# cropinghigh/sdrpp-dvbs-demodulator

Measured on NVIDIA B200. Metric: decoded_info_gbit_s, higher is better.
Workload: dtype int8

## Files before the change

sdrpp-dvbs-demodulator_b200/csrc/ldpc_v2.cuh:

```cuda
#pragma once
#include "ldpc_decoder.cuh"
#include "ldpc_variants.h"

#include <type_traits>

namespace s2 {
namespace v2 {

constexpr int kThreads = 360;

__device__ __forceinline__ uint32_t prmt(uint32_t a, uint32_t b, uint32_t sel) {
    uint32_t d;
    asm("prmt.b32 %0, %1, %2, %3;" : "=r"(d) : "r"(a), "r"(b), "r"(sel));
    return d;
}
__device__ __forceinline__ uint32_t minu2(uint32_t a, uint32_t b) {
    uint32_t d;
    asm("min.u16x2 %0, %1, %2;" : "=r"(d) : "r"(a), "r"(b));
    return d;
}
__device__ __forceinline__ uint32_t min3u2(uint32_t a, uint32_t b, uint32_t c) {
    uint32_t d;
    asm("{.reg .b32 t; min.u16x2 t, %1, %2; min.u16x2 %0, t, %3;}" : "=r"(d) : "r"(a), "r"(b), "r"(c));
    return d;
// ... 242 lines not shown
    const int8_t* ptB = inB + K;
    const int cols = min(360, (K / q) & ~7);
    const int jj = tid % 360, i0 = tid / 360;
    for (int j0 = 0; j0 < 360; j0 += cols) {
        const int nc = min(cols, 360 - j0);
        const int b8 = q * j0 / 8;
        for (int x = tid; x < q * nc / 8; x += THREADS) v4[x] = interleave8(ld_in8<STREAMED>(ptA, b8 + x), ld_in8<STREAMED>(ptB, b8 + x));
        __syncthreads();
        if (jj < nc)
            for (int i = i0; i < q; i += THREADS / 360) __stcg(&wpty[i * 360 + j0 + jj], vdata[jj * q + i]);
        __syncthreads();
    }
    for (int x = tid; x < K / 8; x += THREADS) v4[x] = interleave8(ld_in8<STREAMED>(inA, x), ld_in8<STREAMED>(inB, x));
}

constexpr unsigned kNoPair = 0xFFFFFFFFu;
template <bool STREAMED>
__device__ __noinline__ unsigned claim_next_pair(const LdpcParams2& p, unsigned npairs) {
    if (*reinterpret_cast<const volatile unsigned*>(p.work_counter) + gridDim.x >= npairs) return kNoPair;
    const unsigned np = atomicAdd(p.work_counter, 1u);
    if (np < npairs) {
        const unsigned f0 = 2u * np, nf = min(2u, (unsigned)p.nframes - f0);
        if (!STREAMED || *reinterpret_cast<const volatile unsigned*>(p.arrived) >= f0 + nf) {
            const size_t b = reinterpret_cast<size_t>(p.llr_in + (size_t)f0 * p.N);
            const size_t lo = b & ~(size_t)15, hi = (b + (size_t)nf * p.N + 15) & ~(size_t)15;
            asm volatile("cp.async.bulk.prefetch.L2.global [%0], %1;" ::"l"(lo), "r"((unsigned)(hi - lo)) : "memory");
        }
    }
    return np;
}

static __device__ __noinline__ bool wait_arrived(const unsigned int* arrived_ptr, unsigned need, long long budget) {
    const volatile unsigned* arrived = arrived_ptr;
    const long long t0 = clock64();
    while (*arrived < need) {
        __nanosleep(500);
        if (clock64() - t0 > budget) return false;
    }
    return true;
}

template <int CNT, bool RAGGED, bool STREAMED, int OCC>
__global__ void __launch_bounds__(kThreads, OCC) ldpc_v2_kernel(const __grid_constant__ LdpcParams2 p) {
    constexpr int SLOTS = CNT + 2;
    constexpr int MW = (SLOTS + 1) / 2;
    constexpr int SG = (SLOTS + 7) / 8;
    static_assert(16 * SG >= 2 * SLOTS + 2, "the message record needs two spare bytes (row level)");
    constexpr int DW = (1 + 2 * CNT + 3) & ~3;
    extern __shared__ __align__(16) uint8_t smem_raw[];
    const int q = p.q, K = p.K, N = p.N, R = p.R;
    uint16_t* vdata = reinterpret_cast<uint16_t*>(smem_raw);
    uint16_t* X = reinterpret_cast<uint16_t*>(smem_raw + (size_t)K * 2);
    uint32_t* desc = reinterpret_cast<uint32_t*>(smem_raw + (size_t)K * 2 + 768);
    __shared__ unsigned int s_pair;
    __shared__ int s_bad[2];

    const int tid = threadIdx.x;
    const int j = tid;
    const uint32_t vbase = (uint32_t)__cvta_generic_to_shared(vdata);
    uint32_t dbase = (uint32_t)__cvta_generic_to_shared(desc);
    uint32_t j2 = 2u * (uint32_t)j;
    uint32_t xaddr = (uint32_t)__cvta_generic_to_shared(X) + j2;
    uint32_t m1 = 0xFFFFFFFFu;
    uint4* wmsg = reinterpret_cast<uint4*>(p.workspace + (size_t)blockIdx.x * p.ws_stride);
    uint16_t* wpty = reinterpret_cast<uint16_t*>(p.workspace + (size_t)blockIdx.x * p.ws_stride + (size_t)q * SG * 360 * 16);
    uint32_t* HD = reinterpret_cast<uint32_t*>(reinterpret_cast<uint8_t*>(wpty) + (((size_t)R * 2 + 15) & ~(size_t)15));
    uint32_t* HP = HD + 2 * p.ngroups * kBitWords;
    {
        volatile uint4* opq = reinterpret_cast<volatile uint4*>(HP + 2 * q * kBitWords + 4) + tid;
// ... 1 lines not shown
        j2 = opq->x; xaddr = opq->y; dbase = opq->z; m1 = opq->w;
    }
    for (int x = tid; x < q * DW; x += kThreads) {
        const int i = x / DW, w = x - i * DW;
        const int loff = p.layer_off[i], cnt = (int)p.layer_off[i + 1] - loff;
        uint32_t v = 0;
        if (w == 0) {
            v = (uint32_t)p.layer_nlev[i] | (uint32_t)p.layer_sync[i] << 8 | (uint32_t)cnt << 16;
        } else if (w <= 2 * CNT) {
            const int c = (w - 1) >> 1;
            const int k = loff + (c < cnt ? c : 0);
            v = ((w - 1) & 1) ? (uint32_t)p.link_add[k] : vbase + 720u * p.link_group[k];
        }
        desc[x] = v;
    }
    const int npairs = (p.nframes + 1) >> 1;

    for (int x = tid; x < 2 * (p.ngroups + q) * kBitWords; x += kThreads) __stcg(&HD[x], 0u);
    __shared__ unsigned int s_next;
    if (tid == 0) s_next = kNoPair;

    for (;;) {
        __syncthreads();
        if (tid == 0) {
            unsigned np = s_next;
            if (np == kNoPair) np = atomicAdd(p.work_counter, 1u);
            s_next = kNoPair;
            if (STREAMED && np < (unsigned)npairs) {
                if (!wait_arrived(p.arrived, min(2u * np + 2u, (unsigned)p.nframes), p.wait_budget)) np |= 0x80000000u;
                __threadfence();
            }
            s_pair = np;
        }
        __syncthreads();
        const unsigned pair_word = s_pair;
        const unsigned pair = pair_word & 0x7FFFFFFFu;
        if (pair >= (unsigned)npairs) break;
        const int fa = 2 * pair, fb = 2 * pair + 1;
        const bool hasB = fb < p.nframes;
        if (STREAMED && (pair_word & 0x80000000u)) {
            if (tid == 0) {
                p.iters_out[fa] = kLdpcItersNoInput;
                if (hasB) p.iters_out[fb] = kLdpcItersNoInput;
            }
            continue;
        }
        const int8_t* inA = p.llr_in + (size_t)fa * N;
        const int8_t* inB = p.llr_in + (size_t)(hasB ? fb : fa) * N;

        load_pair<STREAMED, kThreads>(p, inA, inB, vdata, wpty);
        uint32_t pown = 0, psec = 0;
        {
            const uint32_t last = __ldcg(wpty + (q - 1) * 360 + j);
            X[j + 1] = (uint16_t)last;
            pown = unpack_lo(last);
            psec = unpack_lo(__ldcg(wpty + (q - 2) * 360 + j));
        }
        if (tid == 0) X[0] = 0xFFFFu;

        int live = hasB ? 3 : 1;
        uint32_t off[CNT];
        uint32_t lw0 = 0;
        auto link_addresses = [&](int i) {
            uint32_t dw[DW];
#pragma unroll
            for (int x = 0; x < DW; x += 4)
                asm volatile("ld.shared.v4.u32 {%0, %1, %2, %3}, [%4];" : "=r"(dw[x]), "=r"(dw[x + 1]), "=r"(dw[x + 2]), "=r"(dw[x + 3])
                             : "r"(dbase + (uint32_t)(i * DW + x) * 4u));
            lw0 = dw[0];
#pragma unroll
            for (int c = 0; c < CNT; ++c)
                off[c] = dw[1 + 2 * c] + addmin_u32(j2 + dw[2 + 2 * c], (uint32_t)-720);
        };
        auto screen = [&]() -> int {
            link_addresses(q - 1);
            const int cnt = (int)(lw0 >> 16);
            uint32_t sx = pown ^ psec, mn = minu2(__vabsdiffu4(pown, kC128), __vabsdiffu4(psec, kC128));
            int nl = 2;
#pragma unroll
            for (int c = 0; c < CNT; ++c) {
                if (!RAGGED || c < cnt) {
                    const uint32_t u = unpack_lo(lds_u16(off[c]));
                    sx ^= u;
                    mn = minu2(mn, __vabsdiffu4(u, kC128));
                    ++nl;
                }
            }
            if (nl & 1) sx ^= kC128;
            int bad = 0;
            if ((sx & 0x80u) || (mn & 0xFFFFu) == 0) bad |= 1;
            if ((sx & 0x800000u) || (mn >> 16) == 0) bad |= 2;
            return bad;
        };

        __syncthreads();
        int scr = screen();
        int res[2] = {-1, -1};
        for (int n = 0;; ++n) {
            int bad = (__syncthreads_or(scr & 1) ? 1 : 0) | (__syncthreads_or(scr & 2) ? 2 : 0);
            if (live & ~bad)
                bad = full_test<kThreads>(p, wpty, HP, HD, reinterpret_cast<const uint4*>(vdata), s_bad);
            int fin = 0;
            for (int f = 0; f < 2; ++f) {
                if (!(live >> f & 1)) continue;
                if (!(bad >> f & 1)) {
                    res[f] = n;
                    fin |= 1 << f;
                } else if (n == p.max_trials) {
                    fin |= 1 << f;
                }
            }
            if (fin) {
                emit_results<kThreads>(p, fin, res, fa, fb, wpty, reinterpret_cast<const uint4*>(vdata));
                if (tid == 0 && s_next == kNoPair) s_next = claim_next_pair<STREAMED>(p, (unsigned)npairs);
                live &= ~fin;
                if (live) __syncthreads();
            }
            if (!live) break;

            auto pass = [&](auto first_tag) {
                constexpr bool FIRST = decltype(first_tag)::value;
                uint32_t mw[MW];
                uint4 nxt[SG];
                uint32_t pnext = 0;
                uint32_t pprev = 0;
#pragma unroll
                for (int x = 0; x < MW; ++x) mw[x] = 0;
                uint4* rp = wmsg + j;
                uint16_t* pp = wpty + j;
                psec = unpack_lo(lds_u16(xaddr));
                pnext = __ldcg(pp);
                if (!FIRST) {
#pragma unroll
                    for (int s = 0; s < SG; ++s) nxt[s] = __ldcg(rp + s * 360);
                }
                uint32_t lev_next = (FIRST && p.layer_nlev[0] > 1) ? (uint32_t)p.row_level[j] << 24 : 0u;
                for (int i = 0; i < q; ++i) {
                    uint32_t keep = lev_next;
                    if (!FIRST) {
#pragma unroll
                        for (int s = 0; s < SG; ++s) {
                            if (4 * s + 0 < MW) mw[4 * s + 0] = nxt[s].x;
                            if (4 * s + 1 < MW) mw[4 * s + 1] = nxt[s].y;
                            if (4 * s + 2 < MW) mw[4 * s + 2] = nxt[s].z;
                            if (4 * s + 3 < MW) mw[4 * s + 3] = nxt[s].w;
                        }
                        keep = nxt[SG - 1].w;
                    }
                    pown = unpack_lo(i == q - 1 ? lds_u16(xaddr + 2) : pnext);
                    if (i + 1 < q) {
                        pnext = __ldcg(pp + 360);
                        if (!FIRST) {
#pragma unroll
                            for (int s = 0; s < SG; ++s) nxt[s] = __ldcg(rp + (SG + s) * 360);
                        }
                    }
                    link_addresses(i);
                    const int cnt = RAGGED ? (int)(lw0 >> 16) : CNT;
                    const int nlev = (int)(lw0 & 0xFFu);
                    if (FIRST) lev_next = (i + 1 < q && p.layer_nlev[i + 1] > 1) ? (uint32_t)p.row_level[(i + 1) * 360 + j] << 24 : 0u;
                    if (nlev == 1) {
                        row_update<CNT, FIRST, RAGGED>(off, cnt, mw, pown, psec, keep, m1);
                        if (lw0 & 0x100u) __syncthreads();
                    } else {
                        const int mylev = (int)(keep >> 24);
                        for (int lvl = 0; lvl < nlev; ++lvl) {
                            if (mylev == lvl) row_update<CNT, FIRST, RAGGED>(off, cnt, mw, pown, psec, keep, m1);
                            __syncthreads();
                        }
                    }
#pragma unroll
                    for (int s = 0; s < SG; ++s) {
                        uint4 o;
                        o.x = (4 * s + 0 < MW) ? mw[4 * s + 0] : 0u;
                        o.y = (4 * s + 1 < MW) ? mw[4 * s + 1] : 0u;
                        o.z = (4 * s + 2 < MW) ? mw[4 * s + 2] : 0u;
                        o.w = (4 * s + 3 < MW) ? mw[4 * s + 3] : 0u;
                        if (s == SG - 1 && 4 * s + 3 >= MW) o.w = keep & 0xFF000000u;
                        __stcg(rp + s * 360, o);
                    }
                    if (i == 0)
                        sts_u16(xaddr, pack_pair(psec));
                    else
                        __stcg(pp - 360, (uint16_t)pack_pair(psec));
                    pprev = psec;
                    psec = pown;
                    rp += SG * 360;
                    pp += 360;
                }
                psec = pprev;
                {
                    const uint16_t pk = (uint16_t)pack_pair(pown);
                    sts_u16(xaddr + 2, pk);
                    __stcg(pp - 360, pk);
                }
            };
            if (n == 0) pass(std::true_type{});
            else pass(std::false_type{});
            __syncthreads();
            scr = screen();
        }
    }
}

}
}

#define S2_V2_K4(c, r) {{v2::ldpc_v2_kernel<c, r, false, (c <= 9 ? 2 : 1)>, v2::ldpc_v2_kernel<c, r, false, (c <= 9 ? 3 : 2)>}, \
                        {v2::ldpc_v2_kernel<c, r, true, (c <= 9 ? 2 : 1)>, v2::ldpc_v2_kernel<c, r, true, (c <= 9 ? 3 : 2)>}}
#define S2_V2_N4 {{nullptr, nullptr}, {nullptr, nullptr}}
#define V2U(c) {c, S2_V2_K4(c, false), S2_V2_N4}
#define V2B(c) {c, S2_V2_K4(c, false), S2_V2_K4(c, true)}
#define V2R(c) {c, S2_V2_N4, S2_V2_K4(c, true)}
```

sdrpp-dvbs-demodulator_b200/csrc/ldpc_v2l.cuh:

```cuda
#pragma once
#include "ldpc_v2.cuh"

namespace s2 {
namespace v2 {

constexpr int kLdpcThreads2 = 720;

template <int NL, bool FIRST, bool RAGGED>
__device__ __forceinline__ void row_update2(const uint32_t (&off)[NL], int cntl, uint32_t (&mw)[(NL + 2) / 2], uint32_t& preg,
                                            uint32_t keep, uint32_t m1, unsigned lanes) {
    constexpr int DH = NL + 1;
    uint32_t tu[DH], a[DH];
    uint32_t sx = ((2 * DH - 1) & 1) ? kC128 : 0u;
#pragma unroll
    for (int s = 0; s < DH; ++s) {
        uint32_t u;
        if (s == 0)
            u = preg;
        else
            u = (!RAGGED || s - 1 < cntl) ? unpack_lo(lds_u16(off[s - 1])) : kC255;
        uint32_t t = u;
        if (!FIRST) {
            const uint32_t beta = (s & 1) ? unpack_hi(mw[s >> 1]) : unpack_lo(mw[s >> 1]);
            t = addmin_relu(u + beta, kM32, kC255);
// ... 45 lines not shown
template <int CNT, bool RAGGED, bool STREAMED>
__global__ void __launch_bounds__(kLdpcThreads2, 1) ldpc_v2l_kernel(const __grid_constant__ LdpcParams2 p) {
    constexpr int T = kLdpcThreads2;
    constexpr int NL = (CNT + 1) / 2;
    constexpr int DH = NL + 1;
    constexpr int MW = (DH + 1) / 2;
    constexpr int SG = (DH + 7) / 8;
    static_assert(16 * SG >= 2 * DH + 2, "the message record needs two spare bytes (row level)");
    constexpr int HW = (2 * NL + 3) & ~3;
    constexpr int DW = 4 + 2 * HW;
    extern __shared__ __align__(16) uint8_t smem_raw[];
    const int q = p.q, K = p.K, N = p.N, R = p.R;
    uint16_t* vdata = reinterpret_cast<uint16_t*>(smem_raw);
    uint16_t* X = reinterpret_cast<uint16_t*>(smem_raw + (size_t)K * 2);
    uint32_t* desc = reinterpret_cast<uint32_t*>(smem_raw + (size_t)K * 2 + 768);
    __shared__ unsigned int s_pair;
    __shared__ int s_bad[2];

    const int tid = threadIdx.x;
    const int h = tid & 1;
    const int j = tid >> 1;
    const unsigned wl = __activemask();
    const int slot_t = 2 * j + h;
    const uint32_t vbase = (uint32_t)__cvta_generic_to_shared(vdata);
    uint32_t dbase = (uint32_t)__cvta_generic_to_shared(desc) + 16u + (uint32_t)h * HW * 4u;
    uint32_t j2 = 2u * (uint32_t)j;
    uint32_t xaddr = (uint32_t)__cvta_generic_to_shared(X) + j2;
    uint32_t m1 = 0xFFFFFFFFu;
    uint4* wmsg = reinterpret_cast<uint4*>(p.workspace + (size_t)blockIdx.x * p.ws_stride);
    uint16_t* wpty = reinterpret_cast<uint16_t*>(p.workspace + (size_t)blockIdx.x * p.ws_stride + (size_t)q * 2 * SG * 360 * 16);
    uint32_t* HD = reinterpret_cast<uint32_t*>(reinterpret_cast<uint8_t*>(wpty) + (((size_t)R * 2 + 15) & ~(size_t)15));
// ... 7 lines not shown
        const int i = x / DW, w = x - i * DW;
        const int loff = p.layer_off[i], cnt = (int)p.layer_off[i + 1] - loff;
        uint32_t v = 0;
        if (w == 0) {
            v = (uint32_t)p.layer_nlev[i] | (uint32_t)p.layer_sync[i] << 8 | (uint32_t)cnt << 16;
        } else if (w >= 4) {
            const int hh = (w - 4) / HW, e = (w - 4) - hh * HW;
            const int s = e >> 1, d = 2 * s + hh;
            if (s < NL) {
                const int k = loff + (d < cnt ? d : 0);
                v = (e & 1) ? (uint32_t)p.link_add[k] : vbase + 720u * p.link_group[k];
            }
        }
        desc[x] = v;
    }
    const int npairs = (p.nframes + 1) >> 1;
    for (int x = tid; x < 2 * (p.ngroups + q) * kBitWords; x += T) __stcg(&HD[x], 0u);
    __shared__ unsigned int s_next;
    if (tid == 0) s_next = kNoPair;

    for (;;) {
        __syncthreads();
        if (tid == 0) {
            unsigned np = s_next;
            if (np == kNoPair) np = atomicAdd(p.work_counter, 1u);
            s_next = kNoPair;
            if (STREAMED && np < (unsigned)npairs) {
                if (!wait_arrived(p.arrived, min(2u * np + 2u, (unsigned)p.nframes), p.wait_budget)) np |= 0x80000000u;
                __threadfence();
            }
            s_pair = np;
        }
        __syncthreads();
        const unsigned pair_word = s_pair;
        const unsigned pair = pair_word & 0x7FFFFFFFu;
        if (pair >= (unsigned)npairs) break;
        const int fa = 2 * pair, fb = 2 * pair + 1;
        const bool hasB = fb < p.nframes;
        if (STREAMED && (pair_word & 0x80000000u)) {
            if (tid == 0) {
                p.iters_out[fa] = kLdpcItersNoInput;
                if (hasB) p.iters_out[fb] = kLdpcItersNoInput;
            }
            continue;
        }
        const int8_t* inA = p.llr_in + (size_t)fa * N;
        const int8_t* inB = p.llr_in + (size_t)(hasB ? fb : fa) * N;

        load_pair<STREAMED, T>(p, inA, inB, vdata, wpty);
        uint32_t preg;
        {
            const uint32_t w = __ldcg(wpty + (q - 1 - h) * 360 + j);
            if (h == 0) X[j + 1] = (uint16_t)w;
            preg = unpack_lo(w);
        }
        if (tid == 0) X[0] = 0xFFFFu;

        int live = hasB ? 3 : 1;
        uint32_t off[NL];
        uint32_t lw0 = 0;
        auto link_addresses = [&](int i) {
            uint32_t dw[HW];
            const uint32_t lb = dbase + (uint32_t)(i * DW) * 4u;
            lw0 = lds_u32(lb - 16u - (uint32_t)h * HW * 4u);
#pragma unroll
            for (int x = 0; x < HW; x += 4)
                asm volatile("ld.shared.v4.u32 {%0, %1, %2, %3}, [%4];" : "=r"(dw[x]), "=r"(dw[x + 1]), "=r"(dw[x + 2]), "=r"(dw[x + 3])
                             : "r"(lb + (uint32_t)x * 4u));
#pragma unroll
            for (int s = 0; s < NL; ++s) off[s] = dw[2 * s] + addmin_u32(j2 + dw[2 * s + 1], (uint32_t)-720);
        };
        auto half_links = [&](int cnt) { return (cnt - h + 1) >> 1; };
        auto screen = [&]() -> int {
            link_addresses(q - 1);
            const int cntl = half_links((int)(lw0 >> 16));
            uint32_t sx = preg, mn = __vabsdiffu4(preg, kC128);
            int nl = 1;
#pragma unroll
            for (int s = 0; s < NL; ++s) {
                if (s < cntl) {
                    const uint32_t u = unpack_lo(lds_u16(off[s]));
                    sx ^= u;
                    mn = minu2(mn, __vabsdiffu4(u, kC128));
                    ++nl;
                }
            }
            if (nl & 1) sx ^= kC128;
            sx ^= __shfl_xor_sync(wl, sx, 1);
            mn = minu2(mn, __shfl_xor_sync(wl, mn, 1));
            int bad = 0;
            if ((sx & 0x80u) || (mn & 0xFFFFu) == 0) bad |= 1;
            if ((sx & 0x800000u) || (mn >> 16) == 0) bad |= 2;
            return bad;
        };

        __syncthreads();
        int scr = screen();
        int res[2] = {-1, -1};
        for (int n = 0;; ++n) {
            int bad = (__syncthreads_or(scr & 1) ? 1 : 0) | (__syncthreads_or(scr & 2) ? 2 : 0);
            if (live & ~bad)
                bad = full_test<T>(p, wpty, HP, HD, reinterpret_cast<const uint4*>(vdata), s_bad);
            int fin = 0;
            for (int f = 0; f < 2; ++f) {
                if (!(live >> f & 1)) continue;
                if (!(bad >> f & 1)) {
                    res[f] = n;
                    fin |= 1 << f;
                } else if (n == p.max_trials) {
                    fin |= 1 << f;
                }
            }
            if (fin) {
                emit_results<T>(p, fin, res, fa, fb, wpty, reinterpret_cast<const uint4*>(vdata));
                if (tid == 0 && s_next == kNoPair) s_next = claim_next_pair<STREAMED>(p, (unsigned)npairs);
                live &= ~fin;
                if (live) __syncthreads();
            }
            if (!live) break;

            auto pass = [&](auto first_tag) {
                constexpr bool FIRST = decltype(first_tag)::value;
                uint32_t mw[MW];
                uint4 nxt[SG];
                uint32_t pnext = 0;
#pragma unroll
                for (int x = 0; x < MW; ++x) mw[x] = 0;
                uint4* rp = wmsg + slot_t;
                uint16_t* pp = wpty + j;
                if (h == 1) preg = unpack_lo(lds_u16(xaddr));
                pnext = __ldcg(pp);
                if (!FIRST) {
#pragma unroll
                    for (int s = 0; s < SG; ++s) nxt[s] = __ldcg(rp + s * 720);
                }
                uint32_t lev_next = (FIRST && p.layer_nlev[0] > 1) ? (uint32_t)p.row_level[j] << 24 : 0u;
                for (int i = 0; i < q; ++i) {
                    uint32_t keep = lev_next;
                    if (!FIRST) {
#pragma unroll
                        for (int s = 0; s < SG; ++s) {
                            if (4 * s + 0 < MW) mw[4 * s + 0] = nxt[s].x;
                            if (4 * s + 1 < MW) mw[4 * s + 1] = nxt[s].y;
                            if (4 * s + 2 < MW) mw[4 * s + 2] = nxt[s].z;
                            if (4 * s + 3 < MW) mw[4 * s + 3] = nxt[s].w;
                        }
                        keep = nxt[SG - 1].w;
                    }
                    if (h == 0)
                        preg = unpack_lo(i == q - 1 ? lds_u16(xaddr + 2) : pnext);
                    if (i + 1 < q) {
                        pnext = __ldcg(pp + 360);
                        if (!FIRST) {
#pragma unroll
                            for (int s = 0; s < SG; ++s) nxt[s] = __ldcg(rp + (SG + s) * 720);
                        }
                    }
                    link_addresses(i);
                    const int cntl = RAGGED ? half_links((int)(lw0 >> 16)) : (h == 0 ? (CNT + 1) / 2 : CNT / 2);
                    const int nlev = (int)(lw0 & 0xFFu);
                    if (FIRST) lev_next = (i + 1 < q && p.layer_nlev[i + 1] > 1) ? (uint32_t)p.row_level[(i + 1) * 360 + j] << 24 : 0u;
                    constexpr bool kPartial = RAGGED || (CNT & 1);
                    if (nlev == 1) {
                        row_update2<NL, FIRST, kPartial>(off, cntl, mw, preg, keep, m1, wl);
                        if (lw0 & 0x100u) __syncthreads();
                    } else {
                        const int mylev = (int)(keep >> 24);
                        for (int lvl = 0; lvl < nlev; ++lvl) {
                            const unsigned lanes = __ballot_sync(wl, mylev == lvl);
                            if (mylev == lvl) row_update2<NL, FIRST, kPartial>(off, cntl, mw, preg, keep, m1, lanes);
                            __syncthreads();
                        }
                    }
#pragma unroll
                    for (int s = 0; s < SG; ++s) {
                        uint4 o;
                        o.x = (4 * s + 0 < MW) ? mw[4 * s + 0] : 0u;
                        o.y = (4 * s + 1 < MW) ? mw[4 * s + 1] : 0u;
                        o.z = (4 * s + 2 < MW) ? mw[4 * s + 2] : 0u;
                        o.w = (4 * s + 3 < MW) ? mw[4 * s + 3] : 0u;
                        if (s == SG - 1 && (4 * s + 3 >= MW || !(DH & 1))) o.w = (o.w & 0x00FFFFFFu) | (keep & 0xFF000000u);
                        __stcg(rp + s * 720, o);
                    }
                    if (h == 1) {
                        if (i == 0)
                            sts_u16(xaddr, pack_pair(preg));
                        else
                            __stcg(pp - 360, (uint16_t)pack_pair(preg));
                    }
                    const uint32_t other = __shfl_xor_sync(wl, preg, 1);
                    if (h == 1 && i + 1 < q) preg = other;
                    rp += 2 * SG * 360;
                    pp += 360;
                }
                if (h == 0) {
                    const uint16_t pk = (uint16_t)pack_pair(preg);
                    sts_u16(xaddr + 2, pk);
                    __stcg(pp - 360, pk);
                }
            };
            if (n == 0) pass(std::true_type{});
            else pass(std::false_type{});
            __syncthreads();
            scr = screen();
        }
    }
}

}
}

#define S2_V2L_K2(c, r) {v2::ldpc_v2l_kernel<c, r, false>, v2::ldpc_v2l_kernel<c, r, true>}
#define S2_V2L_N2 {nullptr, nullptr}
#define V2LU(c) {c, S2_V2L_K2(c, false), S2_V2L_N2}
#define V2LR(c) {c, S2_V2L_N2, S2_V2L_K2(c, true)}
```

Before: 23.70.

## Refill finished frame lanes independently instead of processing frames in fixed pairs

The LDPC decoder kernel previously claimed two frames at once and iterated until both converged, so a lane whose frame finished early sat idle. Work is now claimed one frame at a time, and a finished lane is refilled with a new frame through a per-lane loader. That loader writes one byte-lane of the interleaved variable and parity storage. A 'fresh' pass kind resets the new lane's check messages, and iteration counts are tracked per lane. This aims to raise useful work per iteration when convergence times vary, at the cost of more control flow, extra single-lane loads, and byte-granular global stores.

```diff
diff --git a/sdrpp-dvbs-demodulator_b200/csrc/ldpc_v2.cuh b/sdrpp-dvbs-demodulator_b200/csrc/ldpc_v2.cuh
--- a/sdrpp-dvbs-demodulator_b200/csrc/ldpc_v2.cuh
+++ b/sdrpp-dvbs-demodulator_b200/csrc/ldpc_v2.cuh
@@ -280,20 +280,54 @@
     for (int x = tid; x < K / 8; x += THREADS) v4[x] = interleave8(ld_in8<STREAMED>(inA, x), ld_in8<STREAMED>(inB, x));
 }
 
-constexpr unsigned kNoPair = 0xFFFFFFFFu;
 template <bool STREAMED>
-__device__ __noinline__ unsigned claim_next_pair(const LdpcParams2& p, unsigned npairs) {
-    if (*reinterpret_cast<const volatile unsigned*>(p.work_counter) + gridDim.x >= npairs) return kNoPair;
-    const unsigned np = atomicAdd(p.work_counter, 1u);
-    if (np < npairs) {
-        const unsigned f0 = 2u * np, nf = min(2u, (unsigned)p.nframes - f0);
-        if (!STREAMED || *reinterpret_cast<const volatile unsigned*>(p.arrived) >= f0 + nf) {
-            const size_t b = reinterpret_cast<size_t>(p.llr_in + (size_t)f0 * p.N);
-            const size_t lo = b & ~(size_t)15, hi = (b + (size_t)nf * p.N + 15) & ~(size_t)15;
-            asm volatile("cp.async.bulk.prefetch.L2.global [%0], %1;" ::"l"(lo), "r"((unsigned)(hi - lo)) : "memory");
-        }
-    }
-    return np;
+__device__ __forceinline__ uint32_t ld_in4(const uint32_t* s) { return STREAMED ? __ldcg(s) : __ldg(s); }
+template <bool STREAMED>
+__device__ __forceinline__ uint32_t ld_in1(const int8_t* s) {
+    return (uint32_t)(uint8_t)(STREAMED ? __ldcg(s) : __ldg(s)) ^ 0x80u;
+}
+
+template <bool STREAMED, int THREADS>
+__device__ __noinline__ void load_lane(const LdpcParams2& p, const int8_t* in, int f, uint16_t* vdata, uint16_t* wpty) {
+    static_assert(THREADS % 360 == 0, "a whole number of threads per column");
+    const int tid = threadIdx.x, q = p.q, K = p.K;
+    const int jj = tid % 360, part = tid / 360;
+    const int s = (K + q * jj) & 3;
+    const uint32_t* src = reinterpret_cast<const uint32_t*>(in + K + q * jj - s);
+    const int nw = (q + s + 3) >> 2;
+    uint8_t* wb = reinterpret_cast<uint8_t*>(wpty) + 2 * jj + f;
+    constexpr int STRIDE = 32 * (THREADS / 360);
+    uint32_t w[9], wn[9];
+    auto load9 = [&](uint32_t (&d)[9], int i0) {
+#pragma unroll
+        for (int t = 0; t < 9; ++t) d[t] = (i0 >> 2) + t < nw ? ld_in4<STREAMED>(src + (i0 >> 2) + t) : 0u;
+    };
+    load9(w, 32 * part);
+    for (int i0 = 32 * part; i0 < q; i0 += STRIDE) {
+        load9(wn, i0 + STRIDE);
+#pragma unroll
+        for (int t = 0; t < 8; ++t) {
+            const uint32_t u = __funnelshift_r(w[t], w[t + 1], 8 * s) ^ 0x80808080u;
+#pragma unroll
+            for (int b = 0; b < 4; ++b)
+                if (i0 + 4 * t + b < q) __stcg(wb + (size_t)(i0 + 4 * t + b) * 720, (uint8_t)(u >> (8 * b)));
+        }
+#pragma unroll
+        for (int t = 0; t < 9; ++t) w[t] = wn[t];
+    }
+    uint4* v4 = reinterpret_cast<uint4*>(vdata);
+    const uint32_t sel_lo = f ? 0x1604u : 0x7150u, sel_hi = f ? 0x3624u : 0x7352u;
+#pragma unroll 4
+    for (int x = tid; x < K / 8; x += THREADS) {
+        const uint2 a = ld_in8<STREAMED>(in, x);
+        const uint32_t ax = a.x ^ 0x80808080u, ay = a.y ^ 0x80808080u;
+        uint4 o = v4[x];
+        o.x = prmt(ax, o.x, sel_lo);
+        o.y = prmt(ax, o.y, sel_hi);
+        o.z = prmt(ay, o.z, sel_lo);
+        o.w = prmt(ay, o.w, sel_hi);
+        v4[x] = o;
+    }
 }
 
 static __device__ __noinline__ bool wait_arrived(const unsigned int* arrived_ptr, unsigned need, long long budget) {
@@ -305,6 +339,60 @@
     }
     return true;
 }
+
+constexpr unsigned kNoFrame = 0xFFFFFFFFu;
+template <bool STREAMED>
+__device__ __noinline__ void take_frames(const LdpcParams2& p, int empty, unsigned* s_new, unsigned* s_next) {
+    const unsigned nframes = (unsigned)p.nframes;
+    unsigned seen = 0;
+    for (int f = 0; f < 2; ++f) {
+        if (!(empty >> f & 1)) continue;
+        unsigned fr;
+        for (;;) {
+            fr = *s_next;
+            *s_next = kNoFrame;
+            if (fr == kNoFrame) fr = atomicAdd(p.work_counter, 1u);
+            seen = max(seen, fr);
+            if (fr >= nframes) {
+                fr = kNoFrame;
+                break;
+            }
+            if (!STREAMED) break;
+            if (wait_arrived(p.arrived, fr + 1u, p.wait_budget)) {
+                __threadfence();
+                break;
+            }
+            p.iters_out[fr] = kLdpcItersNoInput;
+        }
+        s_new[f] = fr;
+    }
+    if (*s_next != kNoFrame || seen + 2u * gridDim.x >= nframes) return;
+    const unsigned fr = atomicAdd(p.work_counter, 1u);
+    *s_next = fr;
+    if (fr < nframes && (!STREAMED || *reinterpret_cast<const volatile unsigned*>(p.arrived) > fr)) {
+        const size_t b = reinterpret_cast<size_t>(p.llr_in + (size_t)fr * p.N);
+        const size_t lo = b & ~(size_t)15, hi = (b + (size_t)p.N + 15) & ~(size_t)15;
+        asm volatile("cp.async.bulk.prefetch.L2.global [%0], %1;" ::"l"(lo), "r"((unsigned)(hi - lo)) : "memory");
+    }
+}
+
+__device__ __forceinline__ int lanes_done(const LdpcParams2& p, int chk, int bad, int n, const int* s_n0, int (&res)[2]) {
+    int fin = 0;
+    for (int f = 0; f < 2; ++f) {
+        res[f] = -1;
+        if (!(chk >> f & 1)) continue;
+        const int it = n - s_n0[f];
+        if (!(bad >> f & 1)) {
+            res[f] = it;
+            fin |= 1 << f;
+        } else if (it == p.max_trials) {
+            fin |= 1 << f;
+        }
+    }
+    return fin;
+}
+
+constexpr int kPassFirst = 0, kPassNext = 1, kPassFresh = 2;
 
 template <int CNT, bool RAGGED, bool STREAMED, int OCC>
 __global__ void __launch_bounds__(kThreads, OCC) ldpc_v2_kernel(const __grid_constant__ LdpcParams2 p) {
@@ -318,7 +406,6 @@
     uint16_t* vdata = reinterpret_cast<uint16_t*>(smem_raw);
     uint16_t* X = reinterpret_cast<uint16_t*>(smem_raw + (size_t)K * 2);
     uint32_t* desc = reinterpret_cast<uint32_t*>(smem_raw + (size_t)K * 2 + 768);
-    __shared__ unsigned int s_pair;
     __shared__ int s_bad[2];
 
     const int tid = threadIdx.x;
@@ -350,192 +437,206 @@
         }
         desc[x] = v;
     }
-    const int npairs = (p.nframes + 1) >> 1;
-
     for (int x = tid; x < 2 * (p.ngroups + q) * kBitWords; x += kThreads) __stcg(&HD[x], 0u);
+    __shared__ unsigned int s_fr[2];
+    __shared__ int s_n0[2];
+    __shared__ unsigned int s_new[2];
     __shared__ unsigned int s_next;
-    if (tid == 0) s_next = kNoPair;
-
-    for (;;) {
+    if (tid == 0) {
+        s_next = kNoFrame;
+        take_frames<STREAMED>(p, 3, s_new, &s_next);
+    }
+
+    uint32_t pown = 0, psec = 0;
+    uint32_t off[CNT];
+    uint32_t lw0 = 0;
+    auto link_addresses = [&](int i) {
+        uint32_t dw[DW];
+#pragma unroll
+        for (int x = 0; x < DW; x += 4)
+            asm volatile("ld.shared.v4.u32 {%0, %1, %2, %3}, [%4];" : "=r"(dw[x]), "=r"(dw[x + 1]), "=r"(dw[x + 2]), "=r"(dw[x + 3])
+                         : "r"(dbase + (uint32_t)(i * DW + x) * 4u));
+        lw0 = dw[0];
+#pragma unroll
+        for (int c = 0; c < CNT; ++c)
+            off[c] = dw[1 + 2 * c] + addmin_u32(j2 + dw[2 + 2 * c], (uint32_t)-720);
+    };
+    auto screen = [&]() -> int {
+        link_addresses(q - 1);
+        const int cnt = (int)(lw0 >> 16);
+        uint32_t sx = pown ^ psec, mn = minu2(__vabsdiffu4(pown, kC128), __vabsdiffu4(psec, kC128));
+        int nl = 2;
+#pragma unroll
+        for (int c = 0; c < CNT; ++c) {
+            if (!RAGGED || c < cnt) {
+                const uint32_t u = unpack_lo(lds_u16(off[c]));
+                sx ^= u;
+                mn = minu2(mn, __vabsdiffu4(u, kC128));
+                ++nl;
+            }
+        }
+        if (nl & 1) sx ^= kC128;
+        int bad = 0;
+        if ((sx & 0x80u) || (mn & 0xFFFFu) == 0) bad |= 1;
+        if ((sx & 0x800000u) || (mn >> 16) == 0) bad |= 2;
+        return bad;
+    };
+
+    int live = 0;
+    int fresh = 0;
+    int empty = 3;
+    int chk = 0;
+    int scr = 0;
+    for (int n = 0;;) {
+        if (empty) {
+            __syncthreads();
+            int got = 0;
+            for (int f = 0; f < 2; ++f)
+                if ((empty >> f & 1) && s_new[f] != kNoFrame) got |= 1 << f;
+            empty = 0;
+            if (!got && !live) break;
+            if (got) {
+                if (!(live & ~got)) {
+                    const int8_t* inA = p.llr_in + (size_t)s_new[(got & 1) ? 0 : 1] * N;
+                    const int8_t* inB = p.llr_in + (size_t)s_new[(got & 2) ? 1 : 0] * N;
+                    load_pair<STREAMED, kThreads>(p, inA, inB, vdata, wpty);
+                    const uint32_t last = __ldcg(wpty + (q - 1) * 360 + j);
+                    X[j + 1] = (uint16_t)last;
+                    pown = unpack_lo(last);
+                    psec = unpack_lo(__ldcg(wpty + (q - 2) * 360 + j));
+                    if (tid == 0) X[0] = 0xFFFFu;
+                } else {
+                    const int f = (got & 1) ? 0 : 1;
+                    const int8_t* in = p.llr_in + (size_t)s_new[f] * N;
+                    load_lane<STREAMED, kThreads>(p, in, f, vdata, wpty);
+                    const uint32_t last = ld_in1<STREAMED>(in + K + q * j + q - 1);
+                    const uint32_t sh = 16u * f, km = ~(0xFFu << sh);
+                    reinterpret_cast<uint8_t*>(X)[2 * j + 2 + f] = (uint8_t)last;
+                    pown = (pown & km) | last << sh;
+                    psec = (psec & km) | ld_in1<STREAMED>(in + K + q * j + q - 2) << sh;
+                    if (tid == 0) reinterpret_cast<uint8_t*>(X)[f] = 0xFFu;
+                }
+                if (tid == 0)
+                    for (int f = 0; f < 2; ++f)
+                        if (got >> f & 1) {
+                            s_fr[f] = s_new[f];
+                            s_n0[f] = n;
+                        }
+                live |= got;
+                fresh |= got;
+                chk = got;
+                __syncthreads();
+                scr = screen();
+            }
+        }
+        if (chk) {
+            int bad = (__syncthreads_or(scr & 1) ? 1 : 0) | (__syncthreads_or(scr & 2) ? 2 : 0);
+            if (chk & ~bad)
+                bad = full_test<kThreads>(p, wpty, HP, HD, reinterpret_cast<const uint4*>(vdata), s_bad);
+            int res[2];
+            const int fin = lanes_done(p, chk, bad, n, s_n0, res);
+            chk = 0;
+            if (fin) {
+                if (tid == 0) take_frames<STREAMED>(p, fin, s_new, &s_next);
+                emit_results<kThreads>(p, fin, res, (int)s_fr[0], (int)s_fr[1], wpty, reinterpret_cast<const uint4*>(vdata));
+                live &= ~fin;
+                fresh &= ~fin;
+                empty = fin;
+                continue;
+            }
+        }
+
+        auto pass = [&](auto kind_tag) {
+            constexpr int KIND = decltype(kind_tag)::value;
+            constexpr bool FIRST = KIND == kPassFirst;
+            const uint32_t km = (fresh & 1) ? 0xFF00FF00u : 0x00FF00FFu;
+            uint32_t mw[MW];
+            uint4 nxt[SG];
+            uint32_t pnext = 0;
+            uint32_t pprev = 0;
+#pragma unroll
+            for (int x = 0; x < MW; ++x) mw[x] = 0;
+            uint4* rp = wmsg + j;
+            uint16_t* pp = wpty + j;
+            psec = unpack_lo(lds_u16(xaddr));
+            pnext = __ldcg(pp);
+            if (!FIRST) {
+#pragma unroll
+                for (int s = 0; s < SG; ++s) nxt[s] = __ldcg(rp + s * 360);
+            }
+            uint32_t lev_next = (FIRST && p.layer_nlev[0] > 1) ? (uint32_t)p.row_level[j] << 24 : 0u;
+            for (int i = 0; i < q; ++i) {
+                uint32_t keep = lev_next;
+                if (!FIRST) {
+#pragma unroll
+                    for (int s = 0; s < SG; ++s) {
+                        if (4 * s + 0 < MW) mw[4 * s + 0] = nxt[s].x;
+                        if (4 * s + 1 < MW) mw[4 * s + 1] = nxt[s].y;
+                        if (4 * s + 2 < MW) mw[4 * s + 2] = nxt[s].z;
+                        if (4 * s + 3 < MW) mw[4 * s + 3] = nxt[s].w;
+                    }
+                    if (KIND == kPassFresh) {
+#pragma unroll
+                        for (int x = 0; x < MW; ++x) mw[x] = (mw[x] & km) | (~km & 0x20202020u);
+                    }
+                    keep = nxt[SG - 1].w;
+                }
+                pown = unpack_lo(i == q - 1 ? lds_u16(xaddr + 2) : pnext);
+                if (i + 1 < q) {
+                    pnext = __ldcg(pp + 360);
+                    if (!FIRST) {
+#pragma unroll
+                        for (int s = 0; s < SG; ++s) nxt[s] = __ldcg(rp + (SG + s) * 360);
+                    }
+                }
+                link_addresses(i);
+                const int cnt = RAGGED ? (int)(lw0 >> 16) : CNT;
+                const int nlev = (int)(lw0 & 0xFFu);
+                if (FIRST) lev_next = (i + 1 < q && p.layer_nlev[i + 1] > 1) ? (uint32_t)p.row_level[(i + 1) * 360 + j] << 24 : 0u;
+                if (nlev == 1) {
+                    row_update<CNT, FIRST, RAGGED>(off, cnt, mw, pown, psec, keep, m1);
+                    if (lw0 & 0x100u) __syncthreads();
+                } else {
+                    const int mylev = (int)(keep >> 24);
+                    for (int lvl = 0; lvl < nlev; ++lvl) {
+                        if (mylev == lvl) row_update<CNT, FIRST, RAGGED>(off, cnt, mw, pown, psec, keep, m1);
+                        __syncthreads();
+                    }
+                }
+#pragma unroll
+                for (int s = 0; s < SG; ++s) {
+                    uint4 o;
+                    o.x = (4 * s + 0 < MW) ? mw[4 * s + 0] : 0u;
+                    o.y = (4 * s + 1 < MW) ? mw[4 * s + 1] : 0u;
+                    o.z = (4 * s + 2 < MW) ? mw[4 * s + 2] : 0u;
+                    o.w = (4 * s + 3 < MW) ? mw[4 * s + 3] : 0u;
+                    if (s == SG - 1 && 4 * s + 3 >= MW) o.w = keep & 0xFF000000u;
+                    __stcg(rp + s * 360, o);
+                }
+                if (i == 0)
+                    sts_u16(xaddr, pack_pair(psec));
+                else
+                    __stcg(pp - 360, (uint16_t)pack_pair(psec));
+                pprev = psec;
+                psec = pown;
+                rp += SG * 360;
+                pp += 360;
+            }
+            psec = pprev;
+            {
+                const uint16_t pk = (uint16_t)pack_pair(pown);
+                sts_u16(xaddr + 2, pk);
+                __stcg(pp - 360, pk);
+            }
+        };
+        if (!(live & ~fresh)) pass(std::integral_constant<int, kPassFirst>{});
+        else if (fresh) pass(std::integral_constant<int, kPassFresh>{});
+        else pass(std::integral_constant<int, kPassNext>{});
+        fresh = 0;
+        ++n;
+        chk = live;
         __syncthreads();
-        if (tid == 0) {
-            unsigned np = s_next;
-            if (np == kNoPair) np = atomicAdd(p.work_counter, 1u);
-            s_next = kNoPair;
-            if (STREAMED && np < (unsigned)npairs) {
-                if (!wait_arrived(p.arrived, min(2u * np + 2u, (unsigned)p.nframes), p.wait_budget)) np |= 0x80000000u;
-                __threadfence();
-            }
-            s_pair = np;
-        }
-        __syncthreads();
-        const unsigned pair_word = s_pair;
-        const unsigned pair = pair_word & 0x7FFFFFFFu;
-        if (pair >= (unsigned)npairs) break;
-        const int fa = 2 * pair, fb = 2 * pair + 1;
-        const bool hasB = fb < p.nframes;
-        if (STREAMED && (pair_word & 0x80000000u)) {
-            if (tid == 0) {
-                p.iters_out[fa] = kLdpcItersNoInput;
-                if (hasB) p.iters_out[fb] = kLdpcItersNoInput;
-            }
-            continue;
-        }
-        const int8_t* inA = p.llr_in + (size_t)fa * N;
-        const int8_t* inB = p.llr_in + (size_t)(hasB ? fb : fa) * N;
-
-        load_pair<STREAMED, kThreads>(p, inA, inB, vdata, wpty);
-        uint32_t pown = 0, psec = 0;
-        {
-            const uint32_t last = __ldcg(wpty + (q - 1) * 360 + j);
-            X[j + 1] = (uint16_t)last;
-            pown = unpack_lo(last);
-            psec = unpack_lo(__ldcg(wpty + (q - 2) * 360 + j));
-        }
-        if (tid == 0) X[0] = 0xFFFFu;
-
-        int live = hasB ? 3 : 1;
-        uint32_t off[CNT];
-        uint32_t lw0 = 0;
-        auto link_addresses = [&](int i) {
-            uint32_t dw[DW];
-#pragma unroll
-            for (int x = 0; x < DW; x += 4)
-                asm volatile("ld.shared.v4.u32 {%0, %1, %2, %3}, [%4];" : "=r"(dw[x]), "=r"(dw[x + 1]), "=r"(dw[x + 2]), "=r"(dw[x + 3])
-                             : "r"(dbase + (uint32_t)(i * DW + x) * 4u));
-            lw0 = dw[0];
-#pragma unroll
-            for (int c = 0; c < CNT; ++c)
-                off[c] = dw[1 + 2 * c] + addmin_u32(j2 + dw[2 + 2 * c], (uint32_t)-720);
-        };
-        auto screen = [&]() -> int {
-            link_addresses(q - 1);
-            const int cnt = (int)(lw0 >> 16);
-            uint32_t sx = pown ^ psec, mn = minu2(__vabsdiffu4(pown, kC128), __vabsdiffu4(psec, kC128));
-            int nl = 2;
-#pragma unroll
-            for (int c = 0; c < CNT; ++c) {
-                if (!RAGGED || c < cnt) {
-                    const uint32_t u = unpack_lo(lds_u16(off[c]));
-                    sx ^= u;
-                    mn = minu2(mn, __vabsdiffu4(u, kC128));
-                    ++nl;
-                }
-            }
-            if (nl & 1) sx ^= kC128;
-            int bad = 0;
-            if ((sx & 0x80u) || (mn & 0xFFFFu) == 0) bad |= 1;
-            if ((sx & 0x800000u) || (mn >> 16) == 0) bad |= 2;
-            return bad;
-        };
-
-        __syncthreads();
-        int scr = screen();
-        int res[2] = {-1, -1};
-        for (int n = 0;; ++n) {
-            int bad = (__syncthreads_or(scr & 1) ? 1 : 0) | (__syncthreads_or(scr & 2) ? 2 : 0);
-            if (live & ~bad)
-                bad = full_test<kThreads>(p, wpty, HP, HD, reinterpret_cast<const uint4*>(vdata), s_bad);
-            int fin = 0;
-            for (int f = 0; f < 2; ++f) {
-                if (!(live >> f & 1)) continue;
-                if (!(bad >> f & 1)) {
-                    res[f] = n;
-                    fin |= 1 << f;
-                } else if (n == p.max_trials) {
-                    fin |= 1 << f;
-                }
-            }
-            if (fin) {
-                emit_results<kThreads>(p, fin, res, fa, fb, wpty, reinterpret_cast<const uint4*>(vdata));
-                if (tid == 0 && s_next == kNoPair) s_next = claim_next_pair<STREAMED>(p, (unsigned)npairs);
-                live &= ~fin;
-                if (live) __syncthreads();
-            }
-            if (!live) break;
-
-            auto pass = [&](auto first_tag) {
-                constexpr bool FIRST = decltype(first_tag)::value;
-                uint32_t mw[MW];
-                uint4 nxt[SG];
-                uint32_t pnext = 0;
-                uint32_t pprev = 0;
-#pragma unroll
-                for (int x = 0; x < MW; ++x) mw[x] = 0;
-                uint4* rp = wmsg + j;
-                uint16_t* pp = wpty + j;
-                psec = unpack_lo(lds_u16(xaddr));
-                pnext = __ldcg(pp);
-                if (!FIRST) {
-#pragma unroll
-                    for (int s = 0; s < SG; ++s) nxt[s] = __ldcg(rp + s * 360);
-                }
-                uint32_t lev_next = (FIRST && p.layer_nlev[0] > 1) ? (uint32_t)p.row_level[j] << 24 : 0u;
-                for (int i = 0; i < q; ++i) {
-                    uint32_t keep = lev_next;
-                    if (!FIRST) {
-#pragma unroll
-                        for (int s = 0; s < SG; ++s) {
-                            if (4 * s + 0 < MW) mw[4 * s + 0] = nxt[s].x;
-                            if (4 * s + 1 < MW) mw[4 * s + 1] = nxt[s].y;
-                            if (4 * s + 2 < MW) mw[4 * s + 2] = nxt[s].z;
-                            if (4 * s + 3 < MW) mw[4 * s + 3] = nxt[s].w;
-                        }
-                        keep = nxt[SG - 1].w;
-                    }
-                    pown = unpack_lo(i == q - 1 ? lds_u16(xaddr + 2) : pnext);
-                    if (i + 1 < q) {
-                        pnext = __ldcg(pp + 360);
-                        if (!FIRST) {
-#pragma unroll
-                            for (int s = 0; s < SG; ++s) nxt[s] = __ldcg(rp + (SG + s) * 360);
-                        }
-                    }
-                    link_addresses(i);
-                    const int cnt = RAGGED ? (int)(lw0 >> 16) : CNT;
-                    const int nlev = (int)(lw0 & 0xFFu);
-                    if (FIRST) lev_next = (i + 1 < q && p.layer_nlev[i + 1] > 1) ? (uint32_t)p.row_level[(i + 1) * 360 + j] << 24 : 0u;
-                    if (nlev == 1) {
-                        row_update<CNT, FIRST, RAGGED>(off, cnt, mw, pown, psec, keep, m1);
-                        if (lw0 & 0x100u) __syncthreads();
-                    } else {
-                        const int mylev = (int)(keep >> 24);
-                        for (int lvl = 0; lvl < nlev; ++lvl) {
-                            if (mylev == lvl) row_update<CNT, FIRST, RAGGED>(off, cnt, mw, pown, psec, keep, m1);
-                            __syncthreads();
-                        }
-                    }
-#pragma unroll
-                    for (int s = 0; s < SG; ++s) {
-                        uint4 o;
-                        o.x = (4 * s + 0 < MW) ? mw[4 * s + 0] : 0u;
-                        o.y = (4 * s + 1 < MW) ? mw[4 * s + 1] : 0u;
-                        o.z = (4 * s + 2 < MW) ? mw[4 * s + 2] : 0u;
-                        o.w = (4 * s + 3 < MW) ? mw[4 * s + 3] : 0u;
-                        if (s == SG - 1 && 4 * s + 3 >= MW) o.w = keep & 0xFF000000u;
-                        __stcg(rp + s * 360, o);
-                    }
-                    if (i == 0)
-                        sts_u16(xaddr, pack_pair(psec));
-                    else
-                        __stcg(pp - 360, (uint16_t)pack_pair(psec));
-                    pprev = psec;
-                    psec = pown;
-                    rp += SG * 360;
-                    pp += 360;
-                }
-                psec = pprev;
-                {
-                    const uint16_t pk = (uint16_t)pack_pair(pown);
-                    sts_u16(xaddr + 2, pk);
-                    __stcg(pp - 360, pk);
-                }
-            };
-            if (n == 0) pass(std::true_type{});
-            else pass(std::false_type{});
-            __syncthreads();
-            scr = screen();
-        }
+        scr = screen();
     }
 }
 
diff --git a/sdrpp-dvbs-demodulator_b200/csrc/ldpc_v2l.cuh b/sdrpp-dvbs-demodulator_b200/csrc/ldpc_v2l.cuh
--- a/sdrpp-dvbs-demodulator_b200/csrc/ldpc_v2l.cuh
+++ b/sdrpp-dvbs-demodulator_b200/csrc/ldpc_v2l.cuh
@@ -83,7 +83,6 @@
     uint16_t* vdata = reinterpret_cast<uint16_t*>(smem_raw);
     uint16_t* X = reinterpret_cast<uint16_t*>(smem_raw + (size_t)K * 2);
     uint32_t* desc = reinterpret_cast<uint32_t*>(smem_raw + (size_t)K * 2 + 768);
-    __shared__ unsigned int s_pair;
     __shared__ int s_bad[2];
 
     const int tid = threadIdx.x;
@@ -121,196 +120,206 @@
         }
         desc[x] = v;
     }
-    const int npairs = (p.nframes + 1) >> 1;
     for (int x = tid; x < 2 * (p.ngroups + q) * kBitWords; x += T) __stcg(&HD[x], 0u);
+    __shared__ unsigned int s_fr[2];
+    __shared__ int s_n0[2];
+    __shared__ unsigned int s_new[2];
     __shared__ unsigned int s_next;
-    if (tid == 0) s_next = kNoPair;
-
-    for (;;) {
+    if (tid == 0) {
+        s_next = kNoFrame;
+        take_frames<STREAMED>(p, 3, s_new, &s_next);
+    }
+
+    uint32_t preg = 0;
+    uint32_t off[NL];
+    uint32_t lw0 = 0;
+    auto link_addresses = [&](int i) {
+        uint32_t dw[HW];
+        const uint32_t lb = dbase + (uint32_t)(i * DW) * 4u;
+        lw0 = lds_u32(lb - 16u - (uint32_t)h * HW * 4u);
+#pragma unroll
+        for (int x = 0; x < HW; x += 4)
+            asm volatile("ld.shared.v4.u32 {%0, %1, %2, %3}, [%4];" : "=r"(dw[x]), "=r"(dw[x + 1]), "=r"(dw[x + 2]), "=r"(dw[x + 3])
+                         : "r"(lb + (uint32_t)x * 4u));
+#pragma unroll
+        for (int s = 0; s < NL; ++s) off[s] = dw[2 * s] + addmin_u32(j2 + dw[2 * s + 1], (uint32_t)-720);
+    };
+    auto half_links = [&](int cnt) { return (cnt - h + 1) >> 1; };
+    auto screen = [&]() -> int {
+        link_addresses(q - 1);
+        const int cntl = half_links((int)(lw0 >> 16));
+        uint32_t sx = preg, mn = __vabsdiffu4(preg, kC128);
+        int nl = 1;
+#pragma unroll
+        for (int s = 0; s < NL; ++s) {
+            if (s < cntl) {
+                const uint32_t u = unpack_lo(lds_u16(off[s]));
+                sx ^= u;
+                mn = minu2(mn, __vabsdiffu4(u, kC128));
+                ++nl;
+            }
+        }
+        if (nl & 1) sx ^= kC128;
+        sx ^= __shfl_xor_sync(wl, sx, 1);
+        mn = minu2(mn, __shfl_xor_sync(wl, mn, 1));
+        int bad = 0;
+        if ((sx & 0x80u) || (mn & 0xFFFFu) == 0) bad |= 1;
+        if ((sx & 0x800000u) || (mn >> 16) == 0) bad |= 2;
+        return bad;
+    };
+
+    int live = 0, fresh = 0, empty = 3, chk = 0, scr = 0;
+    for (int n = 0;;) {
+        if (empty) {
+            __syncthreads();
+            int got = 0;
+            for (int f = 0; f < 2; ++f)
+                if ((empty >> f & 1) && s_new[f] != kNoFrame) got |= 1 << f;
+            empty = 0;
+            if (!got && !live) break;
+            if (got) {
+                if (!(live & ~got)) {
+                    const int8_t* inA = p.llr_in + (size_t)s_new[(got & 1) ? 0 : 1] * N;
+                    const int8_t* inB = p.llr_in + (size_t)s_new[(got & 2) ? 1 : 0] * N;
+                    load_pair<STREAMED, T>(p, inA, inB, vdata, wpty);
+                    const uint32_t w = __ldcg(wpty + (q - 1 - h) * 360 + j);
+                    if (h == 0) X[j + 1] = (uint16_t)w;
+                    preg = unpack_lo(w);
+                    if (tid == 0) X[0] = 0xFFFFu;
+                } else {
+                    const int f = (got & 1) ? 0 : 1;
+                    const int8_t* in = p.llr_in + (size_t)s_new[f] * N;
+                    load_lane<STREAMED, T>(p, in, f, vdata, wpty);
+                    const uint32_t w = ld_in1<STREAMED>(in + K + q * j + q - 1 - h);
+                    const uint32_t sh = 16u * f;
+                    if (h == 0) reinterpret_cast<uint8_t*>(X)[2 * j + 2 + f] = (uint8_t)w;
+                    preg = (preg & ~(0xFFu << sh)) | w << sh;
+                    if (tid == 0) reinterpret_cast<uint8_t*>(X)[f] = 0xFFu;
+                }
+                if (tid == 0)
+                    for (int f = 0; f < 2; ++f)
+                        if (got >> f & 1) {
+                            s_fr[f] = s_new[f];
+                            s_n0[f] = n;
+                        }
+                live |= got;
+                fresh |= got;
+                chk = got;
+                __syncthreads();
+                scr = screen();
+            }
+        }
+        if (chk) {
+            int bad = (__syncthreads_or(scr & 1) ? 1 : 0) | (__syncthreads_or(scr & 2) ? 2 : 0);
+            if (chk & ~bad)
+                bad = full_test<T>(p, wpty, HP, HD, reinterpret_cast<const uint4*>(vdata), s_bad);
+            int res[2];
+            const int fin = lanes_done(p, chk, bad, n, s_n0, res);
+            chk = 0;
+            if (fin) {
+                if (tid == 0) take_frames<STREAMED>(p, fin, s_new, &s_next);
+                emit_results<T>(p, fin, res, (int)s_fr[0], (int)s_fr[1], wpty, reinterpret_cast<const uint4*>(vdata));
+                live &= ~fin;
+                fresh &= ~fin;
+                empty = fin;
+                continue;
+            }
+        }
+
+        auto pass = [&](auto kind_tag) {
+            constexpr int KIND = decltype(kind_tag)::value;
+            constexpr bool FIRST = KIND == kPassFirst;
+            const uint32_t km = (fresh & 1) ? 0xFF00FF00u : 0x00FF00FFu;
+            uint32_t mw[MW];
+            uint4 nxt[SG];
+            uint32_t pnext = 0;
+#pragma unroll
+            for (int x = 0; x < MW; ++x) mw[x] = 0;
+            uint4* rp = wmsg + slot_t;
+            uint16_t* pp = wpty + j;
+            if (h == 1) preg = unpack_lo(lds_u16(xaddr));
+            pnext = __ldcg(pp);
+            if (!FIRST) {
+#pragma unroll
+                for (int s = 0; s < SG; ++s) nxt[s] = __ldcg(rp + s * 720);
+            }
+            uint32_t lev_next = (FIRST && p.layer_nlev[0] > 1) ? (uint32_t)p.row_level[j] << 24 : 0u;
+            for (int i = 0; i < q; ++i) {
+                uint32_t keep = lev_next;
+                if (!FIRST) {
+#pragma unroll
+                    for (int s = 0; s < SG; ++s) {
+                        if (4 * s + 0 < MW) mw[4 * s + 0] = nxt[s].x;
+                        if (4 * s + 1 < MW) mw[4 * s + 1] = nxt[s].y;
+                        if (4 * s + 2 < MW) mw[4 * s + 2] = nxt[s].z;
+                        if (4 * s + 3 < MW) mw[4 * s + 3] = nxt[s].w;
+                    }
+                    if (KIND == kPassFresh) {
+#pragma unroll
+                        for (int x = 0; x < MW; ++x) mw[x] = (mw[x] & km) | (~km & 0x20202020u);
+                    }
+                    keep = nxt[SG - 1].w;
+                }
+                if (h == 0)
+                    preg = unpack_lo(i == q - 1 ? lds_u16(xaddr + 2) : pnext);
+                if (i + 1 < q) {
+                    pnext = __ldcg(pp + 360);
+                    if (!FIRST) {
+#pragma unroll
+                        for (int s = 0; s < SG; ++s) nxt[s] = __ldcg(rp + (SG + s) * 720);
+                    }
+                }
+                link_addresses(i);
+                const int cntl = RAGGED ? half_links((int)(lw0 >> 16)) : (h == 0 ? (CNT + 1) / 2 : CNT / 2);
+                const int nlev = (int)(lw0 & 0xFFu);
+                if (FIRST) lev_next = (i + 1 < q && p.layer_nlev[i + 1] > 1) ? (uint32_t)p.row_level[(i + 1) * 360 + j] << 24 : 0u;
+                constexpr bool kPartial = RAGGED || (CNT & 1);
+                if (nlev == 1) {
+                    row_update2<NL, FIRST, kPartial>(off, cntl, mw, preg, keep, m1, wl);
+                    if (lw0 & 0x100u) __syncthreads();
+                } else {
+                    const int mylev = (int)(keep >> 24);
+                    for (int lvl = 0; lvl < nlev; ++lvl) {
+                        const unsigned lanes = __ballot_sync(wl, mylev == lvl);
+                        if (mylev == lvl) row_update2<NL, FIRST, kPartial>(off, cntl, mw, preg, keep, m1, lanes);
+                        __syncthreads();
+                    }
+                }
+#pragma unroll
+                for (int s = 0; s < SG; ++s) {
+                    uint4 o;
+                    o.x = (4 * s + 0 < MW) ? mw[4 * s + 0] : 0u;
+                    o.y = (4 * s + 1 < MW) ? mw[4 * s + 1] : 0u;
+                    o.z = (4 * s + 2 < MW) ? mw[4 * s + 2] : 0u;
+                    o.w = (4 * s + 3 < MW) ? mw[4 * s + 3] : 0u;
+                    if (s == SG - 1 && (4 * s + 3 >= MW || !(DH & 1))) o.w = (o.w & 0x00FFFFFFu) | (keep & 0xFF000000u);
+                    __stcg(rp + s * 720, o);
+                }
+                if (h == 1) {
+                    if (i == 0)
+                        sts_u16(xaddr, pack_pair(preg));
+                    else
+                        __stcg(pp - 360, (uint16_t)pack_pair(preg));
+                }
+                const uint32_t other = __shfl_xor_sync(wl, preg, 1);
+                if (h == 1 && i + 1 < q) preg = other;
+                rp += 2 * SG * 360;
+                pp += 360;
+            }
+            if (h == 0) {
+                const uint16_t pk = (uint16_t)pack_pair(preg);
+                sts_u16(xaddr + 2, pk);
+                __stcg(pp - 360, pk);
+            }
+        };
+        if (!(live & ~fresh)) pass(std::integral_constant<int, kPassFirst>{});
+        else if (fresh) pass(std::integral_constant<int, kPassFresh>{});
+        else pass(std::integral_constant<int, kPassNext>{});
+        fresh = 0;
+        ++n;
+        chk = live;
         __syncthreads();
-        if (tid == 0) {
-            unsigned np = s_next;
-            if (np == kNoPair) np = atomicAdd(p.work_counter, 1u);
-            s_next = kNoPair;
-            if (STREAMED && np < (unsigned)npairs) {
-                if (!wait_arrived(p.arrived, min(2u * np + 2u, (unsigned)p.nframes), p.wait_budget)) np |= 0x80000000u;
-                __threadfence();
-            }
-            s_pair = np;
-        }
-        __syncthreads();
-        const unsigned pair_word = s_pair;
-        const unsigned pair = pair_word & 0x7FFFFFFFu;
-        if (pair >= (unsigned)npairs) break;
-        const int fa = 2 * pair, fb = 2 * pair + 1;
-        const bool hasB = fb < p.nframes;
-        if (STREAMED && (pair_word & 0x80000000u)) {
-            if (tid == 0) {
-                p.iters_out[fa] = kLdpcItersNoInput;
-                if (hasB) p.iters_out[fb] = kLdpcItersNoInput;
-            }
-            continue;
-        }
-        const int8_t* inA = p.llr_in + (size_t)fa * N;
-        const int8_t* inB = p.llr_in + (size_t)(hasB ? fb : fa) * N;
-
-        load_pair<STREAMED, T>(p, inA, inB, vdata, wpty);
-        uint32_t preg;
-        {
-            const uint32_t w = __ldcg(wpty + (q - 1 - h) * 360 + j);
-            if (h == 0) X[j + 1] = (uint16_t)w;
-            preg = unpack_lo(w);
-        }
-        if (tid == 0) X[0] = 0xFFFFu;
-
-        int live = hasB ? 3 : 1;
-        uint32_t off[NL];
-        uint32_t lw0 = 0;
-        auto link_addresses = [&](int i) {
-            uint32_t dw[HW];
-            const uint32_t lb = dbase + (uint32_t)(i * DW) * 4u;
-            lw0 = lds_u32(lb - 16u - (uint32_t)h * HW * 4u);
-#pragma unroll
-            for (int x = 0; x < HW; x += 4)
-                asm volatile("ld.shared.v4.u32 {%0, %1, %2, %3}, [%4];" : "=r"(dw[x]), "=r"(dw[x + 1]), "=r"(dw[x + 2]), "=r"(dw[x + 3])
-                             : "r"(lb + (uint32_t)x * 4u));
-#pragma unroll
-            for (int s = 0; s < NL; ++s) off[s] = dw[2 * s] + addmin_u32(j2 + dw[2 * s + 1], (uint32_t)-720);
-        };
-        auto half_links = [&](int cnt) { return (cnt - h + 1) >> 1; };
-        auto screen = [&]() -> int {
-            link_addresses(q - 1);
-            const int cntl = half_links((int)(lw0 >> 16));
-            uint32_t sx = preg, mn = __vabsdiffu4(preg, kC128);
-            int nl = 1;
-#pragma unroll
-            for (int s = 0; s < NL; ++s) {
-                if (s < cntl) {
-                    const uint32_t u = unpack_lo(lds_u16(off[s]));
-                    sx ^= u;
-                    mn = minu2(mn, __vabsdiffu4(u, kC128));
-                    ++nl;
-                }
-            }
-            if (nl & 1) sx ^= kC128;
-            sx ^= __shfl_xor_sync(wl, sx, 1);
-            mn = minu2(mn, __shfl_xor_sync(wl, mn, 1));
-            int bad = 0;
-            if ((sx & 0x80u) || (mn & 0xFFFFu) == 0) bad |= 1;
-            if ((sx & 0x800000u) || (mn >> 16) == 0) bad |= 2;
-            return bad;
-        };
-
-        __syncthreads();
-        int scr = screen();
-        int res[2] = {-1, -1};
-        for (int n = 0;; ++n) {
-            int bad = (__syncthreads_or(scr & 1) ? 1 : 0) | (__syncthreads_or(scr & 2) ? 2 : 0);
-            if (live & ~bad)
-                bad = full_test<T>(p, wpty, HP, HD, reinterpret_cast<const uint4*>(vdata), s_bad);
-            int fin = 0;
-            for (int f = 0; f < 2; ++f) {
-                if (!(live >> f & 1)) continue;
-                if (!(bad >> f & 1)) {
-                    res[f] = n;
-                    fin |= 1 << f;
-                } else if (n == p.max_trials) {
-                    fin |= 1 << f;
-                }
-            }
-            if (fin) {
-                emit_results<T>(p, fin, res, fa, fb, wpty, reinterpret_cast<const uint4*>(vdata));
-                if (tid == 0 && s_next == kNoPair) s_next = claim_next_pair<STREAMED>(p, (unsigned)npairs);
-                live &= ~fin;
-                if (live) __syncthreads();
-            }
-            if (!live) break;
-
-            auto pass = [&](auto first_tag) {
-                constexpr bool FIRST = decltype(first_tag)::value;
-                uint32_t mw[MW];
-                uint4 nxt[SG];
-                uint32_t pnext = 0;
-#pragma unroll
-                for (int x = 0; x < MW; ++x) mw[x] = 0;
-                uint4* rp = wmsg + slot_t;
-                uint16_t* pp = wpty + j;
-                if (h == 1) preg = unpack_lo(lds_u16(xaddr));
-                pnext = __ldcg(pp);
-                if (!FIRST) {
-#pragma unroll
-                    for (int s = 0; s < SG; ++s) nxt[s] = __ldcg(rp + s * 720);
-                }
-                uint32_t lev_next = (FIRST && p.layer_nlev[0] > 1) ? (uint32_t)p.row_level[j] << 24 : 0u;
-                for (int i = 0; i < q; ++i) {
-                    uint32_t keep = lev_next;
-                    if (!FIRST) {
-#pragma unroll
-                        for (int s = 0; s < SG; ++s) {
-                            if (4 * s + 0 < MW) mw[4 * s + 0] = nxt[s].x;
-                            if (4 * s + 1 < MW) mw[4 * s + 1] = nxt[s].y;
-                            if (4 * s + 2 < MW) mw[4 * s + 2] = nxt[s].z;
-                            if (4 * s + 3 < MW) mw[4 * s + 3] = nxt[s].w;
-                        }
-                        keep = nxt[SG - 1].w;
-                    }
-                    if (h == 0)
-                        preg = unpack_lo(i == q - 1 ? lds_u16(xaddr + 2) : pnext);
-                    if (i + 1 < q) {
-                        pnext = __ldcg(pp + 360);
-                        if (!FIRST) {
-#pragma unroll
-                            for (int s = 0; s < SG; ++s) nxt[s] = __ldcg(rp + (SG + s) * 720);
-                        }
-                    }
-                    link_addresses(i);
-                    const int cntl = RAGGED ? half_links((int)(lw0 >> 16)) : (h == 0 ? (CNT + 1) / 2 : CNT / 2);
-                    const int nlev = (int)(lw0 & 0xFFu);
-                    if (FIRST) lev_next = (i + 1 < q && p.layer_nlev[i + 1] > 1) ? (uint32_t)p.row_level[(i + 1) * 360 + j] << 24 : 0u;
-                    constexpr bool kPartial = RAGGED || (CNT & 1);
-                    if (nlev == 1) {
-                        row_update2<NL, FIRST, kPartial>(off, cntl, mw, preg, keep, m1, wl);
-                        if (lw0 & 0x100u) __syncthreads();
-                    } else {
-                        const int mylev = (int)(keep >> 24);
-                        for (int lvl = 0; lvl < nlev; ++lvl) {
-                            const unsigned lanes = __ballot_sync(wl, mylev == lvl);
-                            if (mylev == lvl) row_update2<NL, FIRST, kPartial>(off, cntl, mw, preg, keep, m1, lanes);
-                            __syncthreads();
-                        }
-                    }
-#pragma unroll
-                    for (int s = 0; s < SG; ++s) {
-                        uint4 o;
-                        o.x = (4 * s + 0 < MW) ? mw[4 * s + 0] : 0u;
-                        o.y = (4 * s + 1 < MW) ? mw[4 * s + 1] : 0u;
-                        o.z = (4 * s + 2 < MW) ? mw[4 * s + 2] : 0u;
-                        o.w = (4 * s + 3 < MW) ? mw[4 * s + 3] : 0u;
-                        if (s == SG - 1 && (4 * s + 3 >= MW || !(DH & 1))) o.w = (o.w & 0x00FFFFFFu) | (keep & 0xFF000000u);
-                        __stcg(rp + s * 720, o);
-                    }
-                    if (h == 1) {
-                        if (i == 0)
-                            sts_u16(xaddr, pack_pair(preg));
-                        else
-                            __stcg(pp - 360, (uint16_t)pack_pair(preg));
-                    }
-                    const uint32_t other = __shfl_xor_sync(wl, preg, 1);
-                    if (h == 1 && i + 1 < q) preg = other;
-                    rp += 2 * SG * 360;
-                    pp += 360;
-                }
-                if (h == 0) {
-                    const uint16_t pk = (uint16_t)pack_pair(preg);
-                    sts_u16(xaddr + 2, pk);
-                    __stcg(pp - 360, pk);
-                }
-            };
-            if (n == 0) pass(std::true_type{});
-            else pass(std::false_type{});
-            __syncthreads();
-            scr = screen();
-        }
+        scr = screen();
     }
 }
 
```

After: 23.41 (median of 6 runs). -1.2%, worse.
